# ericzzj1989/BALF

Measured on AMD Instinct MI355X. Metric: images/sec + keypoints/sec on 1080p gray (detector forward + NMS + top-K); NMS index match vs CPU ref, higher is better.
Workload: dtype f16 MFMA, split hi+lo operands (3 products), f32 accumulate/LN/GELU/softmax/NMS

## Files before the change

### balf_amd/csrc/stage1_f16.h

```cpp
#pragma once

constexpr int kS1C = 32;
#ifndef BALF_S1_SPLIT_MIX
#define BALF_S1_SPLIT_MIX 2
#endif
typedef float f16v __attribute__((ext_vector_type(16)));

__device__ __forceinline__ f16v mfma32(h8 a, h8 b, f16v c) { return __builtin_amdgcn_mfma_f32_32x32x16_f16(a, b, c, 0, 0, 0); }

constexpr int kS1BtPlane = kS1C * 128;
constexpr int kS1BtBytes = 2 * kS1BtPlane;
__device__ __forceinline__ int s1_bt_wr32(int c, int n) { return c * 128 + (((n >> 2) ^ (c & 7)) << 4) + (n & 3) * 4; }
__device__ __forceinline__ int s1_bt_rd(int c, int j) { return c * 128 + ((j ^ (c & 7)) << 4); }
__device__ __forceinline__ int s1_bt_wr(int c, int li) { return c * 128 + (((li >> 1) ^ (c & 7)) << 4) + (li & 1) * 8; }
#ifndef BALF_GELU_LUT
#define BALF_GELU_LUT 1
#endif
constexpr int kS1LutBytes = BALF_GELU_LUT ? ((kGeluLutN + 1) * 8 + 15) / 16 * 16 : 0;
constexpr int kS1Conv0 = kS1LutBytes;
constexpr int kS1Q1 = kS1Conv0 + 512;
constexpr int kS1D1 = kS1Q1 + 2 * 2048;
constexpr int kS1Mix = kS1D1 + 4 * 2048;
constexpr int kS1D2 = kS1Mix + 8 * 2048;
constexpr int kS1Q2 = kS1D2 + 2 * 2048;
constexpr int kS1R1 = kS1Q2 + 4 * 2048;
constexpr int kS1R2 = kS1R1 + 2 * 2048;
template <int MODE> constexpr int s1_weight_bytes() { return MODE == 0 ? kS1Q2 : kS1R2 + 2 * 2048; }
enum S1Par { kS1pConv0B = 0, kS1pQ1B = 32, kS1pD1B = 64, kS1pGlnG = 128, kS1pGlnB = 160, kS1pMixB1 = 192, kS1pD2B = 256,
             kS1pQ2B = 288, kS1pR1B = 320, kS1pR2B = 352, kS1pLut = 384, kS1ParFloats = 640 };
#ifndef BALF_S1_NW0
#define BALF_S1_NW0 8
#endif
#ifndef BALF_S1_NW1
#define BALF_S1_NW1 8
#endif
#ifndef BALF_S1_NW2
#define BALF_S1_NW2 12
#endif
template <int MODE> constexpr int s1_waves() { return MODE == 0 ? BALF_S1_NW0 : MODE == 1 ? BALF_S1_NW1 : BALF_S1_NW2; }
template <int MODE> constexpr int s1_lds_bytes() {
    return s1_weight_bytes<MODE>() + kS1ParFloats * 4 + (MODE == 2 ? 0 : s1_waves<MODE>() * kS1BtBytes);
}

__device__ __forceinline__ HL s1_split8(const f16v &t, int s) {
    HL o;
    h2 h, l;
#pragma unroll
    for (int i = 0; i < 4; ++i) {
        split_pair<BALF_S1_SPLIT_MIX>(t[8 * s + 2 * i], t[8 * s + 2 * i + 1], h, l);
        o.hi[2 * i] = h[0]; o.hi[2 * i + 1] = h[1]; o.lo[2 * i] = l[0]; o.lo[2 * i + 1] = l[1];
    }
    return o;
}

__device__ __forceinline__ void half_allreduce2(float &s, float &ss) {
    auto swap32 = [](unsigned a, unsigned b) { return __builtin_amdgcn_permlane32_swap(a, b, false, false); };
    auto u = [](float v) { return __builtin_bit_cast(unsigned, v); };
    auto f = [](unsigned v) { return __builtin_bit_cast(float, v); };
    const auto r0 = swap32(u(s), u(ss));
    const float c = f(r0[0]) + f(r0[1]);
    unsigned c1 = u(c);
    asm("" : "+v"(c1));
    const auto r1 = swap32(u(c), c1);
    s = f(r1[0]);
    ss = f(r1[1]);
}

__device__ __forceinline__ void ln_stats32(const f16v &x, float &rstd, float &shift) {
    constexpr float inv_c = 1.0f / 32;
    float s = x[0], ss = x[0] * x[0];
#pragma unroll
    for (int r = 1; r < 16; ++r) {
        s += x[r];
        ss = fmaf(x[r], x[r], ss);
    }
    half_allreduce2(s, ss);
    const float mean = s * inv_c;
    const float var = fmaf(ss, inv_c, -mean * mean);
    rstd = __builtin_amdgcn_rsqf(max0(var) + kLnEps);
    shift = -mean * rstd;
}

__device__ __forceinline__ void s1_ln_split(const f16v (&x)[2], HL (&b)[2][2]) {
#pragma unroll
    for (int p = 0; p < 2; ++p) {
        float rstd, shift;
        ln_stats32(x[p], rstd, shift);
        f16v y;
#pragma unroll
        for (int r = 0; r < 16; ++r) y[r] = fmaf(x[p][r], rstd, shift);
        b[p][0] = s1_split8(y, 0);
        b[p][1] = s1_split8(y, 1);
    }
}

__device__ __forceinline__ void s1_split(const f16v (&x)[2], HL (&b)[2][2]) {
#pragma unroll
    for (int p = 0; p < 2; ++p) {
        b[p][0] = s1_split8(x[p], 0);
        b[p][1] = s1_split8(x[p], 1);
    }
}

template <int KS>
__device__ __forceinline__ void s1_linear(f16v (&acc)[2], const unsigned char *wl, const HL (&b)[2][KS]) {
    HL a[KS];
#pragma unroll
    for (int s = 0; s < KS; ++s) {
        a[s].hi = *reinterpret_cast<const h8 *>(wl + s * 2048);
        a[s].lo = *reinterpret_cast<const h8 *>(wl + s * 2048 + 1024);
    }
#pragma unroll
    for (int s = 0; s < KS; ++s)
#pragma unroll
        for (int p = 0; p < 2; ++p) if (!BALF_DROP_WLO) acc[p] = mfma32(a[s].lo, b[p][s].hi, acc[p]);
#pragma unroll
    for (int s = 0; s < KS; ++s)
#pragma unroll
        for (int p = 0; p < 2; ++p) acc[p] = mfma32(a[s].hi, b[p][s].lo, acc[p]);
#pragma unroll
    for (int s = 0; s < KS; ++s)
#pragma unroll
        for (int p = 0; p < 2; ++p) acc[p] = mfma32(a[s].hi, b[p][s].hi, acc[p]);
}

__device__ __forceinline__ void s1_bias(f16v (&t)[2], const float *par, int h) {
#pragma unroll
    for (int g = 0; g < 4; ++g) {
        const f4 b = *reinterpret_cast<const f4 *>(par + 8 * g + 4 * h);
#pragma unroll
        for (int r = 0; r < 4; ++r) { t[0][4 * g + r] = b[r]; t[1][4 * g + r] = b[r]; }
    }
}

template <int N>
__device__ __forceinline__ void relu32(f16v (&t)[N]) {
#pragma unroll
    for (int p = 0; p < N; ++p)
#pragma unroll
        for (int r = 0; r < 16; ++r) t[p][r] = max0(t[p][r]);
}

template <int N>
__device__ __forceinline__ void lrelu32(f16v (&t)[N]) {
#pragma unroll
    for (int p = 0; p < N; ++p)
#pragma unroll
        for (int r = 0; r < 16; ++r) {
            float v = t[p][r];
            const float m = 0.2f * v;
            asm("v_max_f32 %0, %0, %1" : "+v"(v) : "v"(m));
            t[p][r] = v;
        }
}

template <int LUTN = kGeluLutN>
__device__ __forceinline__ unsigned gelu_lut_off(float x, float magic) {
    static_assert((LUTN + 1) * 8 <= 0x8000, "the byte offset mask below is 15 bits");
    const float y = __builtin_amdgcn_fmed3f(fmaf(x, 0.5f / kGeluLutL, 0.5f), 0.0f, 1.0f);
    const float t = fmaf(y, 8.0f * LUTN, magic);
    return __builtin_bit_cast(unsigned, t) & 0x7FF8u;
}

#ifndef BALF_S1_GELU_CH
#define BALF_S1_GELU_CH 8
#endif
template <int CH, int LUTN = kGeluLutN>
__device__ __forceinline__ void gelu_lut_pipe(f16v (&t)[2], float magic) {
    constexpr int NCH = 32 / CH;
    typedef const f2 __attribute__((address_space(3))) *lds_f2_ptr;
    float v[32];
#pragma unroll
    for (int i = 0; i < 32; ++i) v[i] = t[i >> 4][i & 15];
    auto fence = [] { __builtin_amdgcn_sched_barrier(0x8 | 0x4); };
    f2 ab[2][CH];
    auto issue = [&](int c, int buf) {
#pragma unroll
        for (int i = 0; i < CH; ++i) ab[buf][i] = *reinterpret_cast<lds_f2_ptr>(gelu_lut_off<LUTN>(v[c * CH + i], magic));
    };
    auto finish = [&](int c, int buf) {
#pragma unroll
        for (int i = 0; i < CH; ++i)
            asm("v_fma_f32 %0, %1, %0, %2" : "+v"(v[c * CH + i]) : "v"(ab[buf][i][1]), "v"(ab[buf][i][0]));
    };
    issue(0, 0);
    fence();
#pragma unroll
    for (int c = 1; c < NCH; ++c) {
        issue(c, c & 1);
        fence();
        finish(c - 1, (c - 1) & 1);
        fence();
    }
    finish(NCH - 1, (NCH - 1) & 1);
#pragma unroll
    for (int i = 0; i < 32; ++i) t[i >> 4][i & 15] = v[i];
}

__device__ __forceinline__ void s1_gelu(f16v (&t)[2]) {
    if (BALF_ABLATE_GELU) return;
#if BALF_GELU_LUT
    float magic = 12582912.0f;
    asm("" : "+v"(magic));
    gelu_lut_pipe<BALF_S1_GELU_CH>(t, magic);
#else
#pragma unroll
    for (int p = 0; p < 2; ++p)
#pragma unroll
        for (int r = 0; r < 16; ++r) t[p][r] = gelu1<false>(t[p][r]);
#endif
}

template <typename T>
__device__ __forceinline__ const T *uniform_ptr(const T *p) {
    const unsigned long long u = reinterpret_cast<unsigned long long>(p);
    const unsigned lo = __builtin_amdgcn_readfirstlane((unsigned)u), hi = __builtin_amdgcn_readfirstlane((unsigned)(u >> 32));
    return reinterpret_cast<const T *>(((unsigned long long)hi << 32) | lo);
}

__device__ __forceinline__ HL load_frag32(const float *base, long pix, int C, int s, int h) {
    const char *p = reinterpret_cast<const char *>(base) + pix * (long)C * 4 + s * 64 + h * 16;
    HL o;
    o.hi = *reinterpret_cast<const h8 *>(p);
    o.lo = *reinterpret_cast<const h8 *>(p + 32);
    return o;
}
__device__ __forceinline__ void store_frag32(float *base, long pix, int C, int s, int h, const HL &v) {
    char *p = reinterpret_cast<char *>(base) + pix * (long)C * 4 + s * 64 + h * 16;
    *reinterpret_cast<h8 *>(p) = v.hi;
    *reinterpret_cast<h8 *>(p + 32) = v.lo;
}

__device__ __forceinline__ long uwin_pix(long pix, int C) {
#if BALF_ABLATE_UWINDOW
    return pix & ((((long)BALF_ABLATE_UWINDOW << 20) / (C * 4)) - 1);
#else
    return pix;
#endif
}

#ifndef BALF_S1_KEEP_X0
#define BALF_S1_KEEP_X0 1
#endif
#if BALF_S1_STRICT
#define BALF_S1_WAIT_IN "s_waitcnt vmcnt(0)"
#define BALF_S1_WAIT_U "s_waitcnt vmcnt(0)"
#else
#define BALF_S1_WAIT_IN "s_waitcnt vmcnt(8)"
#define BALF_S1_WAIT_U "s_waitcnt vmcnt(2)"
#endif
template <int MODE, bool U8>
__global__ __launch_bounds__(s1_waves<MODE>() * 64, 1) void stage1_kernel16(StageArgs A) {
    constexpr int C = kS1C, P = 2, NW = s1_waves<MODE>(), NTHR = NW * 64;
    constexpr int BM = MODE == 0 ? 0 : 1;
    constexpr bool TAIL = MODE == 2;
    constexpr bool NEXT32 = kFmt32[1];
    constexpr int STAMP_KID = BM; (void)STAMP_KID;
    STAMP_DECL;
    extern __shared__ __attribute__((aligned(16))) unsigned char smem_raw[];
    float *par = reinterpret_cast<float *>(smem_raw + s1_weight_bytes<MODE>());
    const int lane = threadIdx.x & 63, n = lane & 31, h = lane >> 5;
    const int wave = __builtin_amdgcn_readfirstlane(threadIdx.x >> 6);
    const float *blob = A.blob;
    const StageOff &S = A.off;
    const BranchOff &Br = S.br[BM];

    {
        auto copy = [&](int dst, int src_floats, int bytes) {
            const char *s = reinterpret_cast<const char *>(blob + src_floats);
            for (int i = threadIdx.x * 16; i < bytes; i += NTHR * 16)
                *reinterpret_cast<uint4 *>(smem_raw + dst + i) = *reinterpret_cast<const uint4 *>(s + i);
        };
        if (BALF_GELU_LUT && !TAIL) copy(0, kLayout.gelu_lut, kS1LutBytes);
        copy(kS1Q1, S.q1_w + BM * (2 * 512), 2 * 2048);
        copy(kS1D1, Br.d1_w, 4 * 2048);
        copy(kS1D2, Br.d2_w, 2 * 2048);
        if (!TAIL) copy(kS1Mix, Br.mix_w, 8 * 2048);
        if (BM == 1) {
            copy(kS1Q2, S.q2_w, 4 * 2048);
            copy(kS1R1, S.r1_w, 2 * 2048);
            copy(kS1R2, S.r2_w, 2 * 2048);
        }
        for (int i = threadIdx.x; i < 64; i += NTHR) {
            const int m = i & 31, hh = i >> 5;
            *reinterpret_cast<float2 *>(smem_raw + kS1Conv0 + i * 8) =
                make_float2(blob[S.conv0_w + m * 3 + hh], hh == 0 ? blob[S.conv0_w + m * 3 + 2] : 0.0f);
        }
        for (int i = threadIdx.x; i < kS1ParFloats; i += NTHR) {
            float v;
            if (i < kS1pQ1B) v = blob[S.conv0_b + i];
            else if (i < kS1pD1B) v = blob[S.q1_b + BM * C + (i - kS1pQ1B)];
            else if (i < kS1pGlnG) v = blob[Br.d1_b + (i - kS1pD1B)];
            else if (i < kS1pGlnB) v = blob[Br.gln_g + (i - kS1pGlnG)];
            else if (i < kS1pMixB1) v = blob[Br.gln_b + (i - kS1pGlnB)];
            else if (i < kS1pD2B) v = blob[Br.mix_b + (i - kS1pMixB1)] + 1.0f;
            else if (i < kS1pQ2B) v = blob[Br.d2_b + (i - kS1pD2B)];
            else if (i < kS1pR1B) v = blob[S.q2_b + (i - kS1pQ2B)];
            else if (i < kS1pR2B) v = blob[S.r1_b + (i - kS1pR1B)];
            else if (i < kS1pLut) v = blob[S.r2_b + (i - kS1pR2B)];
            else v = blob[kLayout.u8_lut + (i - kS1pLut)];
            par[i] = v;
        }
        __syncthreads();
    }

    unsigned char *bT = smem_raw + s1_weight_bytes<MODE>() + kS1ParFloats * 4 + wave * kS1BtBytes;
    const unsigned char *wl = smem_raw + lane * 16;

    const int H = A.H, W = A.W, fh = H / 8, fw = W / 8;
    const int per_img = fh * fw;
    const int total = A.B * per_img;
    const int nx = (gridDim.x >> 3) * NW;
    const int wx = (blockIdx.x >> 3) * NW + wave, xcd = blockIdx.x & 7;

    struct Pos { int n, gy, gx; };
    struct Geo { int n, y, x0; long pix0; };
    const int ty_ = n >> 2, tx0_ = 2 * (n & 3);
    const int pstep = (MODE == 0) ? fw : 1;
    auto decompose = [&](int i) {
        Pos c;
        c.n = i / per_img;
        const int rem = i - c.n * per_img;
        c.gy = rem / fw;
        c.gx = rem - c.gy * fw;
        c.n = __builtin_amdgcn_readfirstlane(c.n);
        c.gy = __builtin_amdgcn_readfirstlane(c.gy);
        c.gx = __builtin_amdgcn_readfirstlane(c.gx);
        return c;
    };
    auto geo = [&](const Pos &c) {
        Geo g;
        g.n = c.n;
        int ty = ty_, tx0 = tx0_;
        if constexpr (MODE == 2) {
            int ln = lane;
            asm volatile("" : "+v"(ln));
            ty = (ln & 31) >> 2;
            tx0 = 2 * (ln & 3);
        }
        if (MODE == 0) { g.y = ty * fh + c.gy; g.x0 = tx0 * fw + c.gx; }
        else           { g.y = 8 * c.gy + ty;  g.x0 = 8 * c.gx + tx0; }
        g.pix0 = ((long)g.n * H + g.y) * W + g.x0;
        return g;
    };
    auto load_raw_u8 = [&](const Geo &g, unsigned (&raw)[4]) {
#pragma unroll
        for (int p = 0; p < P; ++p) {
            const int yy = g.y - A.u8_top, xx = g.x0 + p * pstep - A.u8_left;
            const bool ok = yy >= 0 && yy < A.u8_h && xx >= 0 && xx < A.u8_w;
            const unsigned char *px8 = A.X8 + (((long)g.n * A.u8_h + (ok ? yy : 0)) * A.u8_w + (ok ? xx : 0)) * A.u8_ch;
            raw[p] = ok ? (unsigned)px8[A.u8_ch == 3 ? h : 0] : 0x100u;
            raw[2 + p] = ok ? (unsigned)px8[A.u8_ch == 3 ? 2 : 0] : 0x100u;
        }
    };
    const int hw = H * W;
    const unsigned offA = (unsigned)(h * hw) * 4u, offB = (unsigned)(2 * hw) * 4u;
    auto issue_raw = [&](const Geo &g, unsigned (&nraw)[4]) {
        const unsigned vo = (unsigned)(g.y * W + g.x0) * 4u;
        const unsigned voA = vo + offA, voB = vo + offB;
        const float *xb = uniform_ptr(A.X + (long)g.n * 3 * (long)hw);
        if constexpr (BM == 1) {
            unsigned long long a, b;
            asm volatile("s_nop 4\n\tglobal_load_dwordx2 %0, %2, %4\n\tglobal_load_dwordx2 %1, %3, %4"
                         : "=&v"(a), "=&v"(b) : "v"(voA), "v"(voB), "s"(xb) : "memory");
            nraw[0] = (unsigned)a; nraw[1] = (unsigned)(a >> 32); nraw[2] = (unsigned)b; nraw[3] = (unsigned)(b >> 32);
        } else {
            const unsigned st = (unsigned)pstep * 4u;
            const unsigned voA1 = voA + st, voB1 = voB + st;
            asm volatile("s_nop 4\n\tglobal_load_dword %0, %4, %8\n\tglobal_load_dword %1, %5, %8\n\t"
                         "global_load_dword %2, %6, %8\n\tglobal_load_dword %3, %7, %8"
                         : "=&v"(nraw[0]), "=&v"(nraw[1]), "=&v"(nraw[2]), "=&v"(nraw[3])
                         : "v"(voA), "v"(voA1), "v"(voB), "v"(voB1), "s"(xb) : "memory");
        }
    };
    auto take_raw = [&](unsigned (&raw)[4], const unsigned (&nraw)[4]) {
        asm volatile(BALF_S1_WAIT_IN "\n\tv_mov_b32 %0, %4\n\tv_mov_b32 %1, %5\n\tv_mov_b32 %2, %6\n\tv_mov_b32 %3, %7"
                     : "+v"(raw[0]), "+v"(raw[1]), "+v"(raw[2]), "+v"(raw[3])
                     : "v"(nraw[0]), "v"(nraw[1]), "v"(nraw[2]), "v"(nraw[3]) : "memory");
    };
    const int stride = 8 * nx;
    const Pos step = decompose(stride);
    auto advance = [&](Pos c) {
        c.gx += step.gx;
        if (c.gx >= fw) { c.gx -= fw; ++c.gy; }
        c.gy += step.gy;
        if (c.gy >= fh) { c.gy -= fh; ++c.n; }
        c.n += step.n;
        c.n = __builtin_amdgcn_readfirstlane(c.n);
        c.gy = __builtin_amdgcn_readfirstlane(c.gy);
        c.gx = __builtin_amdgcn_readfirstlane(c.gx);
        return c;
    };
    int item = xcd * nx + wx;
    Pos nxt = decompose(item);
    unsigned raw[4] = {}, nraw[4] = {};
    if (!U8 && !TAIL && item < total) {
        issue_raw(geo(nxt), nraw);
        asm volatile("s_waitcnt vmcnt(0)" ::: "memory");
    }
    const float2 a0 = *reinterpret_cast<const float2 *>(smem_raw + kS1Conv0 + lane * 8);

    unsigned long long sat = 0;
    for (; item < total; item += stride) {
        const Geo g = geo(nxt);
        if (item + stride < total) nxt = advance(nxt);
        const long pix0 = g.pix0;
        if (U8 && !TAIL) load_raw_u8(g, raw);
        f16v x1t[TAIL ? 2 : 1];
        f4 sct[4];
        if constexpr (TAIL) {
#pragma unroll
            for (int gq = 0; gq < 4; ++gq) {
#pragma unroll
                for (int p = 0; p < P; ++p) {
                    const f4 v = *reinterpret_cast<const f4 *>(A.R + (long)item * (64 * C) + ((p * 4 + gq) * 64 + lane) * 4);
#pragma unroll
                    for (int r = 0; r < 4; ++r) x1t[p][4 * gq + r] = v[r];
                }
            }
        }
        STAMP(0);
        float bx[4];
        auto make_bx = [&]() {
#pragma unroll
            for (int i = 0; i < 4; ++i) {
                if (U8) bx[i] = raw[i] < 256u ? par[kS1pLut + (raw[i] & 255u)] : 0.0f;
                else bx[i] = __builtin_bit_cast(float, raw[i]);
            }
        };
        if constexpr (!TAIL) {
            if constexpr (!U8) {
                take_raw(raw, nraw);
            }
            make_bx();
        }
        HL ub[(MODE == 1) ? P : 1][2];
        if constexpr (MODE == 1) {
            if constexpr (U8) {
#pragma unroll
                for (int p = 0; p < P; ++p) { ub[p][0] = load_frag32(A.U, pix0 + p * pstep, C, 0, h); ub[p][1] = load_frag32(A.U, pix0 + p * pstep, C, 1, h); }
            } else {
#if BALF_ABLATE_UWINDOW
                const unsigned uoff = (unsigned)uwin_pix((long)g.n * hw + g.y * W + g.x0, 32) * 128u + h * 16u;
                const char *ubase = uniform_ptr(reinterpret_cast<const char *>(A.U));
#else
                const unsigned uoff = (unsigned)(g.y * W + g.x0) * 128u + h * 16u;
                const char *ubase = uniform_ptr(reinterpret_cast<const char *>(A.U) + (long)g.n * (long)hw * 128);
#endif
#define BALF_S1_UB(PI, SI)                                                                                          \
    asm volatile("s_nop 4\n\tglobal_load_dwordx4 %0, %2, %3 offset:%c4\n\tglobal_load_dwordx4 %1, %2, %3 offset:%c5"        \
                 : "=&v"(ub[PI][SI].hi), "=&v"(ub[PI][SI].lo) : "v"(uoff), "s"(ubase), "i"(PI * 128 + SI * 64), "i"(PI * 128 + SI * 64 + 32) : "memory")
                BALF_S1_UB(0, 0); BALF_S1_UB(0, 1); BALF_S1_UB(1, 0); BALF_S1_UB(1, 1);
#undef BALF_S1_UB
            }
        }
        if constexpr (!U8 && !TAIL) issue_raw(geo(nxt), nraw);
        STAMP(1);
        auto conv0 = [&](f16v (&x0v)[2]) {
            s1_bias(x0v, par + kS1pConv0B, h);
#pragma unroll
            for (int p = 0; p < P; ++p) {
                x0v[p] = __builtin_amdgcn_mfma_f32_32x32x2f32(a0.x, bx[p], x0v[p], 0, 0, 0);
                x0v[p] = __builtin_amdgcn_mfma_f32_32x32x2f32(a0.y, bx[2 + p], x0v[p], 0, 0, 0);
            }
            relu32(x0v);
        };

        HL b[P][2];
        if constexpr (TAIL) {
            s1_ln_split(x1t, b);
            f16v m1[2];
            s1_bias(m1, par + kS1pR1B, h);
            s1_linear<2>(m1, wl + kS1R1, b);
            lrelu32(m1);
            s1_split(m1, b);
            f16v t[2];
            s1_bias(t, par + kS1pR2B, h);
            s1_linear<2>(t, wl + kS1R2, b);
            if constexpr (U8) load_raw_u8(g, raw);
            else {
                const float *xp = A.X + (long)g.n * 3 * (long)hw + (long)g.y * W + g.x0;
                const float2 va = *reinterpret_cast<const float2 *>(xp + (long)h * hw), vb = *reinterpret_cast<const float2 *>(xp + 2L * hw);
                raw[0] = __builtin_bit_cast(unsigned, va.x); raw[1] = __builtin_bit_cast(unsigned, va.y);
                raw[2] = __builtin_bit_cast(unsigned, vb.x); raw[3] = __builtin_bit_cast(unsigned, vb.y);
            }
            make_bx();
            f16v x0v[2];
            conv0(x0v);
#pragma unroll
            for (int p = 0; p < P; ++p)
#pragma unroll
                for (int r = 0; r < 16; ++r) x0v[p][r] = x1t[p][r] + x0v[p][r];
            asm volatile("" ::: "memory");
#pragma unroll
            for (int gq = 0; gq < 4; ++gq) sct[gq] = *reinterpret_cast<const f4 *>(A.scale + (long)g.n * C + 8 * gq + 4 * h);
            f16v mx;
#pragma unroll
            for (int r = 0; r < 16; ++r) {
                const float sc = sct[r >> 2][r & 3];
                const float v0 = fmaf(t[0][r], sc, x0v[0][r]);
                const float v1 = fmaf(t[1][r], sc, x0v[1][r]);
                const float m = __builtin_fmaxf(v0, v1);
                const int mi = __builtin_bit_cast(int, m);
                const int up = __builtin_amdgcn_update_dpp(0, mi, 0x104 , 0xF, 0xF, false);
                const int pv = __builtin_amdgcn_update_dpp(up, mi, 0x114 , 0xF, 0xA, false);
                mx[r] = __builtin_fmaxf(m, __builtin_bit_cast(float, pv));
            }
#pragma unroll
            for (int r = 0; r < 16; ++r) sat |= __builtin_amdgcn_ballot_w64(__builtin_fabsf(mx[r]) >= kF16Max);
            {
                const long opix = ((long)g.n * (H / 2) + (g.y >> 1)) * (W / 2) + (g.x0 >> 1);
                const HL s0 = s1_split8(mx, 0), s1 = s1_split8(mx, 1);
                const int part = (n >> 2) & 1;
                const unsigned pm = 0u - (unsigned)part;
                typedef unsigned u4 __attribute__((ext_vector_type(4)));
                auto pick = [&](const h8 &a, const h8 &b) {
                    const u4 ua = __builtin_bit_cast(u4, a), ub = __builtin_bit_cast(u4, b);
                    u4 o;
#pragma unroll
                    for (int i = 0; i < 4; ++i) o[i] = (ub[i] & pm) | (ua[i] & ~pm);
                    return __builtin_bit_cast(h8, o);
                };
                if constexpr (NEXT32) {
                    const HL v{pick(s0.hi, s1.hi), pick(s0.lo, s1.lo)};
                    store_frag32(A.out, opix, C, part, h, v);
                } else {
                    typedef _Float16 h4 __attribute__((ext_vector_type(4)));
                    auto lo4 = [](const h8 &v) { return h4{v[0], v[1], v[2], v[3]}; };
                    auto hi4 = [](const h8 &v) { return h4{v[4], v[5], v[6], v[7]}; };
                    auto cat = [](const h4 &a, const h4 &c) { return h8{a[0], a[1], a[2], a[3], c[0], c[1], c[2], c[3]}; };
                    char *op = reinterpret_cast<char *>(A.out) + opix * (long)C * 4 + (h + 2 * part) * 16;
                    *reinterpret_cast<h8 *>(op) = pick(cat(lo4(s0.hi), lo4(s1.hi)), cat(hi4(s0.hi), hi4(s1.hi)));
                    *reinterpret_cast<h8 *>(op + 64) = pick(cat(lo4(s0.lo), lo4(s1.lo)), cat(hi4(s0.lo), hi4(s1.lo)));
                }
            }
        } else {
        f16v x0k[(MODE == 1 && BALF_S1_KEEP_X0) ? 2 : 1];
        if constexpr (MODE == 1 && BALF_S1_KEEP_X0) {
            conv0(x0k);
            s1_ln_split(x0k, b);
        } else {
            f16v x0v[2];
            conv0(x0v);
            s1_ln_split(x0v, b);
        }
        STAMP(2);
        f16v z[2];
        s1_bias(z, par + kS1pQ1B, h);
        s1_linear<2>(z, wl + kS1Q1, b);
        s1_gelu(z);
        STAMP(3);
        s1_ln_split(z, b);
        STAMP(4);

        f16v ga[2];
        s1_bias(ga, par + kS1pD1B, h);
        s1_linear<2>(ga, wl + kS1D1, b);
        s1_gelu(ga);
        STAMP(5);
        {
            f16v gb[2];
            s1_bias(gb, par + kS1pD1B + C, h);
            s1_linear<2>(gb, wl + kS1D1 + 2 * 2048, b);
            s1_gelu(gb);
            float rstd[P], shift[P];
#pragma unroll
            for (int p = 0; p < P; ++p) ln_stats32(gb[p], rstd[p], shift[p]);
#pragma unroll
            for (int gq = 0; gq < 4; ++gq) {
                const f4 gg = *reinterpret_cast<const f4 *>(par + kS1pGlnG + 8 * gq + 4 * h);
                const f4 bb = *reinterpret_cast<const f4 *>(par + kS1pGlnB + 8 * gq + 4 * h);
#pragma unroll
                for (int r = 0; r < 4; ++r) {
                    const float v0 = fmaf(fmaf(gb[0][4 * gq + r], rstd[0], shift[0]), gg[r], bb[r]);
                    const float v1 = fmaf(fmaf(gb[1][4 * gq + r], rstd[1], shift[1]), gg[r], bb[r]);
                    h2 hh, ll;
                    split_pair<BALF_S1_SPLIT_MIX>(v0, v1, hh, ll);
                    unsigned char *row = bT + s1_bt_wr32(8 * gq + 4 * h + r, n);
                    *reinterpret_cast<h2 *>(row) = hh;
                    *reinterpret_cast<h2 *>(row + kS1BtPlane) = ll;
                }
            }
        }
        STAMP(6);
        {
            HL a[4];
#pragma unroll
            for (int s = 0; s < 4; ++s) {
                const unsigned char *row = bT + s1_bt_rd(n, 2 * s + h);
                a[s].hi = *reinterpret_cast<const h8 *>(row);
                a[s].lo = *reinterpret_cast<const h8 *>(row + kS1BtPlane);
            }
            const float2 mb1 = *reinterpret_cast<const float2 *>(par + kS1pMixB1 + 2 * n);
#pragma unroll
            for (int pt = 0; pt < P; ++pt) {
                const float mb = pt ? mb1.y : mb1.x;
                f16v m;
#pragma unroll
                for (int r = 0; r < 16; ++r) m[r] = mb;
#pragma unroll
                for (int s = 0; s < 4; ++s) {
                    HL w;
                    w.hi = *reinterpret_cast<const h8 *>(wl + kS1Mix + (pt * 4 + s) * 2048);
                    w.lo = *reinterpret_cast<const h8 *>(wl + kS1Mix + (pt * 4 + s) * 2048 + 1024);
                    m = mfma32(a[s].lo, w.hi, m);
                    m = mfma32(a[s].hi, w.lo, m);
                    m = mfma32(a[s].hi, w.hi, m);
                }
#pragma unroll
                for (int r = 0; r < 16; ++r) ga[pt][r] *= m[r];
            }
        }
        STAMP(7);
        s1_split(ga, b);
        f16v o[2];
        s1_bias(o, par + kS1pD2B, h);
        s1_linear<2>(o, wl + kS1D2, b);
#pragma unroll
        for (int p = 0; p < P; ++p)
#pragma unroll
            for (int r = 0; r < 16; ++r) o[p][r] += z[p][r];

        STAMP(8);
        if constexpr (MODE == 0) {
#pragma unroll
            for (int p = 0; p < P; ++p) {
                store_frag32(A.U, uwin_pix(pix0 + p * pstep, C), C, 0, h, s1_split8(o[p], 0));
                store_frag32(A.U, uwin_pix(pix0 + p * pstep, C), C, 1, h, s1_split8(o[p], 1));
            }
            STAMP(9);
        } else {
            s1_split(o, b);
            f16v x1[2];
            s1_bias(x1, par + kS1pQ2B, h);
            s1_linear<2>(x1, wl + kS1Q2 + 2 * 2048, b);
            if constexpr (!U8)
                asm volatile(BALF_S1_WAIT_U
                             : "+v"(ub[0][0].hi), "+v"(ub[0][0].lo), "+v"(ub[0][1].hi), "+v"(ub[0][1].lo), "+v"(ub[1][0].hi),
                               "+v"(ub[1][0].lo), "+v"(ub[1][1].hi), "+v"(ub[1][1].lo) :: "memory");
            s1_linear<2>(x1, wl + kS1Q2, ub);
            STAMP(9);
            {
#if BALF_S1_KEEP_X0
                f16v (&x0v)[2] = x0k;
#else
                f16v x0v[2];
                conv0(x0v);
#endif
#pragma unroll
                for (int p = 0; p < P; ++p) {
#pragma unroll
                    for (int r = 0; r < 16; ++r) x1[p][r] += x0v[p][r];
#pragma unroll
                    for (int gq = 0; gq < 4; ++gq)
                        *reinterpret_cast<f4 *>(A.R + (long)item * (64 * C) + ((p * 4 + gq) * 64 + lane) * 4) =
                            f4{x1[p][4 * gq], x1[p][4 * gq + 1], x1[p][4 * gq + 2], x1[p][4 * gq + 3]};
                }
            }
            STAMP(10);
            s1_ln_split(x1, b);
            f16v m1[2];
            s1_bias(m1, par + kS1pR1B, h);
            s1_linear<2>(m1, wl + kS1R1, b);
            lrelu32(m1);
            {
                float cs[8];
#pragma unroll
                for (int r = 0; r < 8; ++r) {
                    const float sa = m1[0][r] + m1[1][r], sb = m1[0][r + 8] + m1[1][r + 8];
                    const auto sw = __builtin_amdgcn_permlane16_swap(__builtin_bit_cast(unsigned, sa), __builtin_bit_cast(unsigned, sb), false, false);
                    unsigned w0 = sw[0], w1 = sw[1];
                    asm("" : "+v"(w0), "+v"(w1));
                    float s = __builtin_bit_cast(float, w0) + __builtin_bit_cast(float, w1);
                    cs[r] = row_ror_add<1>(row_ror_add<2>(row_ror_add<4>(row_ror_add<8>(s))));
                }
                if ((lane & 15) == 0) {
                    const int row = lane >> 4, c0 = 16 * (row & 1) + 4 * (row >> 1);
                    float *pp = A.partial + (long)item * C + c0;
                    *reinterpret_cast<f4 *>(pp) = f4{cs[0], cs[1], cs[2], cs[3]};
                    *reinterpret_cast<f4 *>(pp + 8) = f4{cs[4], cs[5], cs[6], cs[7]};
                }
            }
            STAMP(12);
        }
        }
    }
    if (TAIL && sat != 0) status_raise(A.status, 1 );
}
```

Before: 910.0.

## Prefetch tail-stage x1 tiles into LDS via async global_load_lds double-step

In the tail mode of stage1, the per-item x1 activation tile is now fetched with asynchronous global-to-LDS loads issued one iteration ahead, then read from the per-wave LDS buffer instead of directly from global memory. The tail mode also gets a compact LDS layout that holds only conv0, R1 and R2 weights and skips copying unused weights (LUT, Q1, D1, D2, mix, Q2). This is meant to hide global load latency behind the previous item's compute. The cost is adding the per-wave staging buffer to tail LDS usage, plus wait-count tuning that could race if the vmcnt assumptions are wrong.

```diff
diff --git a/balf_amd/csrc/stage1_f16.h b/balf_amd/csrc/stage1_f16.h
--- a/balf_amd/csrc/stage1_f16.h
+++ b/balf_amd/csrc/stage1_f16.h
@@ -25,7 +25,10 @@
 constexpr int kS1Q2 = kS1D2 + 2 * 2048;
 constexpr int kS1R1 = kS1Q2 + 4 * 2048;
 constexpr int kS1R2 = kS1R1 + 2 * 2048;
-template <int MODE> constexpr int s1_weight_bytes() { return MODE == 0 ? kS1Q2 : kS1R2 + 2 * 2048; }
+constexpr int kS1TConv0 = 0;
+constexpr int kS1TR1 = kS1TConv0 + 512;
+constexpr int kS1TR2 = kS1TR1 + 2 * 2048;
+template <int MODE> constexpr int s1_weight_bytes() { return MODE == 0 ? kS1Q2 : MODE == 1 ? kS1R2 + 2 * 2048 : kS1TR2 + 2 * 2048; }
 enum S1Par { kS1pConv0B = 0, kS1pQ1B = 32, kS1pD1B = 64, kS1pGlnG = 128, kS1pGlnB = 160, kS1pMixB1 = 192, kS1pD2B = 256,
              kS1pQ2B = 288, kS1pR1B = 320, kS1pR2B = 352, kS1pLut = 384, kS1ParFloats = 640 };
 #ifndef BALF_S1_NW0
@@ -39,7 +42,7 @@
 #endif
 template <int MODE> constexpr int s1_waves() { return MODE == 0 ? BALF_S1_NW0 : MODE == 1 ? BALF_S1_NW1 : BALF_S1_NW2; }
 template <int MODE> constexpr int s1_lds_bytes() {
-    return s1_weight_bytes<MODE>() + kS1ParFloats * 4 + (MODE == 2 ? 0 : s1_waves<MODE>() * kS1BtBytes);
+    return s1_weight_bytes<MODE>() + kS1ParFloats * 4 + s1_waves<MODE>() * kS1BtBytes;
 }
 
 __device__ __forceinline__ HL s1_split8(const f16v &t, int s) {
@@ -245,9 +248,11 @@
 #if BALF_S1_STRICT
 #define BALF_S1_WAIT_IN "s_waitcnt vmcnt(0)"
 #define BALF_S1_WAIT_U "s_waitcnt vmcnt(0)"
+#define BALF_S1_WAIT_X1 "s_waitcnt vmcnt(0)"
 #else
 #define BALF_S1_WAIT_IN "s_waitcnt vmcnt(8)"
 #define BALF_S1_WAIT_U "s_waitcnt vmcnt(2)"
+#define BALF_S1_WAIT_X1 "s_waitcnt vmcnt(2)"
 #endif
 template <int MODE, bool U8>
 __global__ __launch_bounds__(s1_waves<MODE>() * 64, 1) void stage1_kernel16(StageArgs A) {
@@ -256,6 +261,7 @@
     constexpr bool TAIL = MODE == 2;
     constexpr bool NEXT32 = kFmt32[1];
     constexpr int STAMP_KID = BM; (void)STAMP_KID;
+    constexpr int oConv0 = TAIL ? kS1TConv0 : kS1Conv0, oR1 = TAIL ? kS1TR1 : kS1R1, oR2 = TAIL ? kS1TR2 : kS1R2;
     STAMP_DECL;
     extern __shared__ __attribute__((aligned(16))) unsigned char smem_raw[];
     float *par = reinterpret_cast<float *>(smem_raw + s1_weight_bytes<MODE>());
@@ -271,19 +277,21 @@
             for (int i = threadIdx.x * 16; i < bytes; i += NTHR * 16)
                 *reinterpret_cast<uint4 *>(smem_raw + dst + i) = *reinterpret_cast<const uint4 *>(s + i);
         };
-        if (BALF_GELU_LUT && !TAIL) copy(0, kLayout.gelu_lut, kS1LutBytes);
-        copy(kS1Q1, S.q1_w + BM * (2 * 512), 2 * 2048);
-        copy(kS1D1, Br.d1_w, 4 * 2048);
-        copy(kS1D2, Br.d2_w, 2 * 2048);
-        if (!TAIL) copy(kS1Mix, Br.mix_w, 8 * 2048);
+        if constexpr (!TAIL) {
+            if (BALF_GELU_LUT) copy(0, kLayout.gelu_lut, kS1LutBytes);
+            copy(kS1Q1, S.q1_w + BM * (2 * 512), 2 * 2048);
+            copy(kS1D1, Br.d1_w, 4 * 2048);
+            copy(kS1D2, Br.d2_w, 2 * 2048);
+            copy(kS1Mix, Br.mix_w, 8 * 2048);
+            if (BM == 1) copy(kS1Q2, S.q2_w, 4 * 2048);
+        }
         if (BM == 1) {
-            copy(kS1Q2, S.q2_w, 4 * 2048);
-            copy(kS1R1, S.r1_w, 2 * 2048);
-            copy(kS1R2, S.r2_w, 2 * 2048);
+            copy(oR1, S.r1_w, 2 * 2048);
+            copy(oR2, S.r2_w, 2 * 2048);
         }
         for (int i = threadIdx.x; i < 64; i += NTHR) {
             const int m = i & 31, hh = i >> 5;
-            *reinterpret_cast<float2 *>(smem_raw + kS1Conv0 + i * 8) =
+            *reinterpret_cast<float2 *>(smem_raw + oConv0 + i * 8) =
                 make_float2(blob[S.conv0_w + m * 3 + hh], hh == 0 ? blob[S.conv0_w + m * 3 + 2] : 0.0f);
         }
         for (int i = threadIdx.x; i < kS1ParFloats; i += NTHR) {
@@ -398,7 +406,23 @@
         issue_raw(geo(nxt), nraw);
         asm volatile("s_waitcnt vmcnt(0)" ::: "memory");
     }
-    const float2 a0 = *reinterpret_cast<const float2 *>(smem_raw + kS1Conv0 + lane * 8);
+    const float2 a0 = *reinterpret_cast<const float2 *>(smem_raw + oConv0 + lane * 8);
+    auto issue_x1 = [&](int it) {
+        typedef __attribute__((address_space(3))) void *lds_ptr;
+        const char *src = reinterpret_cast<const char *>(A.R) + (long)it * (64 * C * 4) + lane * 16;
+        constexpr int NT = 2;
+#pragma unroll
+        for (int half = 0; half < 2; ++half) {
+            __builtin_amdgcn_global_load_lds(src + half * 4096, (lds_ptr)(bT + half * 4096), 16, 0, NT);
+            __builtin_amdgcn_global_load_lds(src + half * 4096, (lds_ptr)(bT + half * 4096), 16, 1024, NT);
+            __builtin_amdgcn_global_load_lds(src + half * 4096, (lds_ptr)(bT + half * 4096), 16, 2048, NT);
+            __builtin_amdgcn_global_load_lds(src + half * 4096, (lds_ptr)(bT + half * 4096), 16, 3072, NT);
+        }
+    };
+    if (TAIL && item < total) {
+        issue_x1(item);
+        asm volatile("s_waitcnt vmcnt(0)" ::: "memory");
+    }
 
     unsigned long long sat = 0;
     for (; item < total; item += stride) {
@@ -409,15 +433,18 @@
         f16v x1t[TAIL ? 2 : 1];
         f4 sct[4];
         if constexpr (TAIL) {
+            asm volatile(BALF_S1_WAIT_X1 ::: "memory");
 #pragma unroll
             for (int gq = 0; gq < 4; ++gq) {
 #pragma unroll
                 for (int p = 0; p < P; ++p) {
-                    const f4 v = *reinterpret_cast<const f4 *>(A.R + (long)item * (64 * C) + ((p * 4 + gq) * 64 + lane) * 4);
+                    const f4 v = *reinterpret_cast<const f4 *>(bT + ((p * 4 + gq) * 64 + lane) * 16);
 #pragma unroll
                     for (int r = 0; r < 4; ++r) x1t[p][4 * gq + r] = v[r];
                 }
             }
+            asm volatile("s_waitcnt lgkmcnt(0)" : "+v"(x1t[0]), "+v"(x1t[1]) :: "memory");
+            if (item + stride < total) issue_x1(item + stride);
         }
         STAMP(0);
         float bx[4];
@@ -471,12 +498,12 @@
             s1_ln_split(x1t, b);
             f16v m1[2];
             s1_bias(m1, par + kS1pR1B, h);
-            s1_linear<2>(m1, wl + kS1R1, b);
+            s1_linear<2>(m1, wl + oR1, b);
             lrelu32(m1);
             s1_split(m1, b);
             f16v t[2];
             s1_bias(t, par + kS1pR2B, h);
-            s1_linear<2>(t, wl + kS1R2, b);
+            s1_linear<2>(t, wl + oR2, b);
             if constexpr (U8) load_raw_u8(g, raw);
             else {
                 const float *xp = A.X + (long)g.n * 3 * (long)hw + (long)g.y * W + g.x0;
```

After: 911.8, median of 2. Within noise of the previous version (+0.2%).
